# loop-Z/omniisaacgymenvs_loop

Measured on NVIDIA B200. Metric: ASV env-steps/sec, higher is better.
Workload: dtype f32

## Files before the change

omniisaacgymenvs_loop_b200/csrc/usv_step.cu:

```cuda
#include "usv_step_core.cuh"

namespace usv {

constexpr int kBlock = 128, kMinB = 7;
constexpr double kResidentL2Share = 0.75;

__device__ __forceinline__ void post_classic(EnvState& e, const EnvConst& k, const UsvStepParams& p, bool do_reset,
                                             bool first_call, const DynOut& s, StepOut& o, const int what = USV_CXY_ALL) {
  const float pxn = s.pxn, pyn = s.pyn, vxn = s.vxn, vyn = s.vyn, wn = s.wn, yawn = s.yawn, hs = s.hs, hc = s.hc;
  const float pa0 = s.pa0, pa1 = s.pa1;
  const float ex = k.tx - pxn, ey = k.ty - pyn;
  const float theta = wrap_pi(yawn);
  const float beta = fast_atan2(ey, ex);
  const float xa = beta - theta + USV_PI_F;
  const float alpha = ((xa >= USV_2PI_F) ? xa - USV_2PI_F : xa) - USV_PI_F;
  const float herr = fabsf(alpha);
  const float d = sqrtf(ex * ex + ey * ey);
  const float inv_d = (d > 0.0f) ? __fdividef(1.0f, d) : 0.0f;
  const float cb = (d > 0.0f) ? ex * inv_d : 1.0f, sb = ey * inv_d;
  const float ca = cb * hc + sb * hs, sa = sb * hc - cb * hs;
  o.obs[0] = hc * vxn + hs * vyn;
  o.obs[1] = -hs * vxn + hc * vyn;
  o.obs[2] = wn;
  o.obs[3] = ca;
  o.obs[4] = sa;
  o.obs[5] = d;
  o.obs[6] = vxn;
  o.obs[7] = vyn;
  o.obs[8] = 0.0f;
  o.obs[9] = vxn;
  o.obs[10] = vyn;
  o.obs[11] = 0.0f;
  o.obs[12] = 0.0f;
  const float speed = sqrtf(vxn * vxn + vyn * vyn);
  const int goal = (d < p.position_tolerance) && (speed < p.goal_speed_gate);
  if (what & USV_CXY_REWARD) e.goal_cnt = e.goal_cnt * goal + goal;
  float dist_rew;
  if (p.reward_mode == USV_REWARD_LINEAR) {
    dist_rew = p.position_scale * (e.prev_d - d);
  } else if (p.reward_mode == USV_REWARD_SQUARE) {
    dist_rew = p.position_scale * (e.prev_d * e.prev_d - d * d);
  } else {
    dist_rew = p.position_scale * (expf(-d / p.exponential_reward_coeff) - expf(-e.prev_d / p.exponential_reward_coeff));
  }
  const float h2 = herr * herr;
  const float align = p.align_la1 * (__expf(p.align_la2 * (h2 * h2)) + __expf(p.align_la3 * h2));
  if (do_reset) dist_rew = 0.0f;
  float speed_rew;
  const float sclamp = 1.0f - fminf(fmaxf(speed / 1.0f, 0.0f), 1.0f);
  if (d > 3.5f) {
    const bool in_range = (speed >= 0.8f) && (speed <= 1.5f);
    const float ds = speed - 1.15f;
    speed_rew = in_range ? 0.1f : __expf(-(ds * ds) * 5.0f) * 0.1f;
  } else if (d > 2.5f) {
    speed_rew = sclamp * 0.15f;
  } else if (d > 1.5f) {
    speed_rew = sclamp * 0.25f;
  } else {
    speed_rew = sclamp * 0.35f;
  }
  if (!(d == d)) speed_rew = 0.0f;
  const float goal_rew = (float)e.goal_cnt * p.goal_reward;
  const float task_rew = dist_rew + align + speed_rew + goal_rew + p.time_reward;
  if (what & USV_CXY_REWARD) e.prev_d = d;
  const float asum = pa0 + pa1;
  const float dw = first_call ? 0.0f : (wn - e.prev_w);
  const float dasum = first_call ? 0.0f : (asum - e.prev_asum);
  float pen_lin = 0.0f, pen_ang = 0.0f, pen_angvar = 0.0f, pen_energy = 0.0f, pen_actvar = 0.0f;
  if (p.pen_linear_vel.form != USV_PEN_OFF) pen_lin = penalty_scalar(p.pen_linear_vel, speed);
  if (p.pen_angular_vel.form != USV_PEN_OFF) pen_ang = penalty_scalar(p.pen_angular_vel, wn);
  if (p.pen_angular_vel_variation.form != USV_PEN_OFF) pen_angvar = penalty_scalar(p.pen_angular_vel_variation, dw);
  if (p.pen_energy.form == USV_PEN_NEG_SUM) pen_energy = -(pa0 + pa1) * p.pen_energy.c1 + p.pen_energy.c2;
  else if (p.pen_energy.form == USV_PEN_EXP_NEG_SUMSQ) pen_energy = (__expf(-(pa0 * pa0 + pa1 * pa1)) - 1.0f) * p.pen_energy.c1;
  if (p.pen_action_variation.form != USV_PEN_OFF) pen_actvar = penalty_scalar(p.pen_action_variation, dasum);
  const float penalties = pen_lin + pen_ang + pen_angvar + pen_energy + pen_actvar;
  if (what & USV_CXY_PENALTY) {
    e.prev_w = wn;
    e.prev_asum = asum;
  }
  o.task_rew = task_rew;
  o.penalty = penalties;
  o.rew = task_rew + penalties;
  int die = (d > p.kill_dist) ? 1 : 0;
  if ((e.goal_cnt >= p.kill_after_n_steps_in_tolerance) && (speed < p.goal_speed_gate)) die = 1;
  o.die = die;
  o.done = (e.progress >= p.max_episode_length - 1) ? 1 : die;
  o.dist_rew = dist_rew; o.align_rew = align; o.speed_rew = speed_rew; o.d = d; o.speed = speed;
  o.bdist = d - p.kill_dist;
  o.bpen = -expf(-o.bdist / 0.25f) * p.boundary_cost;
  o.pen_lin = pen_lin; o.pen_ang = pen_ang; o.pen_angvar = pen_angvar; o.pen_energy = pen_energy; o.pen_actvar = pen_actvar;
  o.absw = fabsf(wn); o.asum = asum;
  float chk = o.rew * 0.0f;
#pragma unroll
  for (int j = 0; j < kObs; ++j) chk = fmaf(o.obs[j], 0.0f, chk);
  o.finite = (chk == 0.0f);
#pragma unroll
  for (int j = 0; j < kObs; ++j)
    if (j != 8 && j != 11 && j != 12) o.obs[j] = fminf(fmaxf(o.obs[j], -p.clip_obs), p.clip_obs);
}

template <int kDisturb, bool kLutGlobal>
__device__ __forceinline__ void control_step(EnvState& e, EnvConst& k, const UsvStepParams& p, bool do_reset,
                                             float2 act, uint64_t gid, int64_t lid, uint64_t step, bool first_call,
                                             const float* __restrict__ s_lutL, const float* __restrict__ s_lutR,
                                             StepOut& o) {
  DynOut s;
  step_dynamics<kDisturb, kLutGlobal>(e, k, p, do_reset, act, gid, lid, step, s_lutL, s_lutR, s);
  post_classic(e, k, p, do_reset, first_call, s, o);
}

__device__ __forceinline__ void accumulate_stats(float* __restrict__ st0, int64_t i0, bool was_reset,
                                                 const StepOut& o, const UsvStepParams& p) {
  float* __restrict__ st = st0 + tile_base(i0, USV_ST_COUNT);
  const float v[USV_ST_COUNT] = {o.dist_rew, o.align_rew, o.speed_rew, o.d, o.speed, o.bpen, o.bdist,
                                 o.pen_lin, o.pen_ang, o.pen_angvar, o.pen_energy, o.pen_actvar,
                                 o.speed, o.absw, o.asum};
#pragma unroll
  for (int f = 0; f < USV_ST_COUNT; ++f) {
    const float prev = was_reset ? 0.0f : st[f * kTile];
    st[f * kTile] = prev + v[f];
  }
}


template <Cache C = Cache::kNormal>
__device__ __forceinline__ void write_obs_tile(float* s_obs, const StepOut& o, bool active, float* __restrict__ obs,
                                               int64_t block_start, int64_t n) {
  const int lane = threadIdx.x & 31, warp = threadIdx.x >> 5;
  float* sw = s_obs + warp * (32 * kObs);
  if (active) {
#pragma unroll
    for (int j = 0; j < kObs; ++j) sw[lane * kObs + j] = o.obs[j];
  }
  __syncwarp();
  const int64_t warp_start = block_start + (int64_t)warp * 32;
  if (warp_start >= n) return;
  const int rows = (int)min((int64_t)32, n - warp_start);
  const int total = rows * kObs;
  float* g = obs + warp_start * kObs;
  if (rows == 32 && (((uintptr_t)g & 15) == 0)) {
    const float4* s4 = reinterpret_cast<const float4*>(sw);
    float4* g4 = reinterpret_cast<float4*>(g);
#pragma unroll
    for (int q = lane; q < (32 * kObs) / 4; q += 32) st<C>(g4 + q, s4[q]);
  } else {
    for (int q = lane; q < total; q += 32) st<C>(g + q, sw[q]);
  }
  __syncwarp();
}

template <int kDisturb, bool kStats, Cache kOnePass>
__global__ void __launch_bounds__(kBlock, kMinB) step_fused_kernel(UsvEnvBuffers b, const float2* __restrict__ actions,
                                                            float* __restrict__ obs, float* __restrict__ rew,
                                                            int64_t n, const __grid_constant__ UsvStepParams p) {
  extern __shared__ __align__(16) float smem[];
  float* s_obs = smem;
  const float* __restrict__ s_lutL = b.lut_left;
  const float* __restrict__ s_lutR = b.lut_right;
  const int64_t block_start = (int64_t)blockIdx.x * kBlock;
  const int64_t i = block_start + threadIdx.x;
  const bool active = i < n;
  EnvState e;
  EnvConst k;
  bool do_reset = false;
  float2 act = make_float2(0.f, 0.f);
  if (active) {
    load_state(b.state, i, e);
    load_consts<kDisturb, kOnePass>(b.consts, i, k);
    do_reset = b.reset_buf[i] != 0;
    act = ld<kOnePass>(actions + i);
  }
  StepOut o;
  if (active) {
    control_step<kDisturb, true>(e, k, p, do_reset, act, (uint64_t)(p.env_id_offset + i), i, p.step_counter + (b.step_offset ? *b.step_offset : 0ull),
                                 p.first_call != 0, s_lutL, s_lutR, o);
    store_state(b.state, i, e);
    if (do_reset) store_consts<kDisturb, kOnePass>(b.consts, i, k);
    if (kStats) accumulate_stats(b.stats, i, do_reset, o, p);
    st<kOnePass>(rew + i, o.rew);
    b.reset_buf[i] = (int64_t)o.done;
    if (b.nonfinite_flag) {
      if (!o.finite) atomicOr(b.nonfinite_flag, 1u);
      if (!isfinite(act.x) || !isfinite(act.y)) atomicOr(b.nonfinite_flag, 2u);
    }
  }
  write_obs_tile<kOnePass>(s_obs, o, active, obs, block_start, n);
}

template <int kDisturb, bool kStats>
__global__ void __launch_bounds__(kBlock) rollout_fused_kernel(UsvEnvBuffers b, const float2* __restrict__ actions,
                                                               float* __restrict__ obs, float* __restrict__ rew,
                                                               int64_t* __restrict__ done, int T, int64_t n,
                                                               const __grid_constant__ UsvStepParams p) {
  extern __shared__ __align__(16) float smem[];
  float* s_obs = smem;
  float* s_lutL = smem + kBlock * kObs;
  float* s_lutR = s_lutL + p.n_lut;
  for (int t = threadIdx.x; t < p.n_lut; t += kBlock) {
    s_lutL[t] = b.lut_left[t];
    s_lutR[t] = b.lut_right[t];
  }
  const int64_t block_start = (int64_t)blockIdx.x * kBlock;
  const int64_t i = block_start + threadIdx.x;
  const bool active = i < n;
  EnvState e;
  EnvConst k;
  bool do_reset = false;
  bool consts_dirty = false;
  if (active) {
    load_state(b.state, i, e);
    load_consts<kDisturb>(b.consts, i, k);
    do_reset = b.reset_buf[i] != 0;
  }
  __syncthreads();
  bool first_call = p.first_call != 0;
  bool bad = false;
  const uint64_t step0 = p.step_counter + (b.step_offset ? *b.step_offset : 0ull);
  for (int t = 0; t < T; ++t) {
    StepOut o;
    if (active) {
      const float2 act = actions[(int64_t)t * n + i];
      control_step<kDisturb, false>(e, k, p, do_reset, act, (uint64_t)(p.env_id_offset + i), i, step0 + (uint64_t)t,
                             first_call, s_lutL, s_lutR, o);
      consts_dirty |= do_reset;
      if (kStats) accumulate_stats(b.stats, i, do_reset, o, p);
      if (rew) rew[(int64_t)t * n + i] = o.rew;
      if (done) done[(int64_t)t * n + i] = (int64_t)o.done;
      bad |= !o.finite || !isfinite(act.x) || !isfinite(act.y);
      do_reset = o.done != 0;
    }
    first_call = false;
    if (obs) {
      write_obs_tile(s_obs, o, active, obs + (int64_t)t * n * kObs, block_start, n);
    }
  }
  if (active) {
    store_state(b.state, i, e);
    if (consts_dirty) store_consts<kDisturb>(b.consts, i, k);
    b.reset_buf[i] = do_reset ? 1 : 0;
    if (b.nonfinite_flag && bad) atomicOr(b.nonfinite_flag, 1u);
  }
}

template <int kDisturb>
__global__ void __launch_bounds__(kBlock) planar_forces_kernel(UsvEnvBuffers b, float* __restrict__ out, int64_t n,
                                                               const __grid_constant__ UsvStepParams p) {
  const int64_t i = (int64_t)blockIdx.x * kBlock + threadIdx.x;
  if (i >= n) return;
  EnvState e;
  EnvConst k;
  load_state(b.state, i, e);
  load_consts<kDisturb>(b.consts, i, k);
  float ox = 0.0f, oy = 0.0f;
  if (kDisturb && p.envs_per_row > 0) {
    ox = p.grid_row_offset - (float)(int)(i / p.envs_per_row) * p.env_spacing;
    oy = (float)(int)(i % p.envs_per_row) * p.env_spacing - p.grid_col_offset;
  }
  float du, dv, dr, Fx, Fy, Tz, ax, ay, rdot, hsn, hcs;
  fsincos(e.psi, &hsn, &hcs);
  planar_wrench<kDisturb>(e, k, p, make_damp(k, p), ox, oy, 1.0f / k.mass, 1.0f / (p.izz * k.kiz), hsn, hcs, du, dv, dr, Fx, Fy, Tz, ax, ay, rdot);
  float* o = out + i * 8;
  o[0] = du; o[1] = dv; o[2] = dr; o[3] = Fx; o[4] = Fy; o[5] = Tz; o[6] = ax; o[7] = ay;
}

static size_t step_smem(const UsvStepParams* p) { return (size_t)(kBlock * kObs + 2 * p->n_lut) * sizeof(float); }
static size_t step_smem_nolut() { return (size_t)(kBlock * kObs) * sizeof(float); }

__global__ void __launch_bounds__(256) capturexy_task_kernel(UsvCaptureXYIO io, int64_t n, UsvStepParams p) {
  const int64_t i = (int64_t)blockIdx.x * blockDim.x + threadIdx.x;
  if (i >= n) return;
  const float2 z2 = make_float2(0.f, 0.f);
  const float2 pos = io.position ? reinterpret_cast<const float2*>(io.position)[i] : z2;
  const float2 hd = io.heading ? reinterpret_cast<const float2*>(io.heading)[i] : make_float2(1.f, 0.f);
  const float2 vel = io.linear_velocity ? reinterpret_cast<const float2*>(io.linear_velocity)[i] : z2;
  const float2 act = io.actions ? reinterpret_cast<const float2*>(io.actions)[i] : z2;
  const float2 tgt = io.target ? reinterpret_cast<const float2*>(io.target)[i] : z2;
  DynOut s;
  s.pxn = pos.x; s.pyn = pos.y; s.vxn = vel.x; s.vyn = vel.y;
  s.wn = io.angular_velocity ? io.angular_velocity[i] : 0.f;
  s.hc = hd.x; s.hs = hd.y;
  s.yawn = fast_atan2(hd.y, hd.x);
  s.pa0 = act.x; s.pa1 = act.y;
  s.raw0 = s.raw1 = s.t0 = s.t1 = s.c0 = s.c1 = 0.f;
  EnvState e;
  e.x = pos.x; e.y = pos.y; e.psi = s.yawn; e.vx = vel.x; e.vy = vel.y; e.r = s.wn; e.thrL = e.thrR = 0.f;
  e.progress = 0;
  e.goal_cnt = io.goal_reached ? io.goal_reached[i] : 0;
  const bool jr = io.just_reset ? io.just_reset[i] != 0 : false;
  EnvConst k;
  k.tx = tgt.x; k.ty = tgt.y;
  if (io.first_reward || !io.prev_position_dist) {
    const float ex = tgt.x - pos.x, ey = tgt.y - pos.y;
    e.prev_d = sqrtf(ex * ex + ey * ey);
  } else {
    e.prev_d = io.prev_position_dist[i];
  }
  e.prev_w = io.prev_angular_velocity ? io.prev_angular_velocity[i] : 0.f;
  e.prev_asum = io.prev_action_sum ? io.prev_action_sum[i] : 0.f;
  p.kill_dist = io.kill_dist;
  p.max_episode_length = 0x7fffffff;
  StepOut o;
  post_classic(e, k, p, jr, io.first_penalty != 0, s, o, io.what);
  if ((io.what & USV_CXY_OBS) && io.obs) {
#pragma unroll
    for (int j = 0; j < kObs; ++j) io.obs[i * kObs + j] = o.obs[j];
  }
  if (io.what & USV_CXY_REWARD) {
    if (io.reward) io.reward[i] = o.task_rew;
    if (io.reward_terms) { io.reward_terms[i * 3] = o.dist_rew; io.reward_terms[i * 3 + 1] = o.align_rew; io.reward_terms[i * 3 + 2] = o.speed_rew; }
    if (io.goal_reached) io.goal_reached[i] = e.goal_cnt;
    if (io.prev_position_dist) io.prev_position_dist[i] = e.prev_d;
  }
  if (io.what & USV_CXY_PENALTY) {
    if (io.penalty) io.penalty[i] = o.penalty;
    if (io.penalty_terms) {
      io.penalty_terms[i * 5] = o.pen_lin; io.penalty_terms[i * 5 + 1] = o.pen_ang; io.penalty_terms[i * 5 + 2] = o.pen_angvar;
      io.penalty_terms[i * 5 + 3] = o.pen_energy; io.penalty_terms[i * 5 + 4] = o.pen_actvar;
    }
    if (io.prev_angular_velocity) io.prev_angular_velocity[i] = e.prev_w;
    if (io.prev_action_sum) io.prev_action_sum[i] = e.prev_asum;
  }
  if ((io.what & USV_CXY_KILLS) && io.die) io.die[i] = o.die;
}

}

using namespace usv;

extern "C" {

int usv_capturexy_obs_reward_done_f32(const UsvCaptureXYIO* io, int64_t n, const UsvStepParams* p, void* stream) {
  if (!io || !p) return USV_E_NULL;
  if (n < 0) return USV_E_SIZE;
  if (n == 0) return USV_OK;
  if (!(io->what & USV_CXY_ALL) || (io->what & ~USV_CXY_ALL)) return USV_E_PARAM;
  if (!io->position || !io->target || !io->linear_velocity) return USV_E_NULL;
  if ((io->what & USV_CXY_OBS) && (!io->obs || !io->heading || !io->angular_velocity)) return USV_E_NULL;
  if ((io->what & USV_CXY_REWARD) && (!io->reward || !io->heading || !io->goal_reached)) return USV_E_NULL;
  if ((io->what & USV_CXY_PENALTY) && (!io->penalty || !io->actions || !io->angular_velocity)) return USV_E_NULL;
  if ((io->what & USV_CXY_KILLS) && (!io->die || !io->goal_reached)) return USV_E_NULL;
  const uintptr_t al = (uintptr_t)io->position | (uintptr_t)io->target | (uintptr_t)io->linear_velocity | (uintptr_t)io->heading |
                       (uintptr_t)io->actions;
  if (al & 7) return USV_E_ALIGN;
  capturexy_task_kernel<<<grid_for(n, 256), 256, 0, (cudaStream_t)stream>>>(*io, n, *p);
  return finish_launch();
}

int usv_step_fused_f32(const UsvEnvBuffers* b, const float* actions, float* obs, float* rew, int64_t n,
                       const UsvStepParams* p, void* stream) {
  int rc = check_common(b, n, p);
  if (rc) return rc;
  if (n == 0) return USV_OK;
  if (!actions || !obs || !rew) return USV_E_NULL;
  if ((uintptr_t)actions & 7) return USV_E_ALIGN;
  const size_t smem = step_smem_nolut();
  const int grid = grid_for(n, kBlock);
  const bool dis = wants_disturb(p), st = b->stats != nullptr;
  cudaStream_t s = (cudaStream_t)stream;
  const double reread = (double)n * (USV_S_COUNT * 4 + 8 + (st ? USV_ST_COUNT * 4 : 0));
  const bool one_pass_cs = reread <= kResidentL2Share * l2_bytes();
#define USV_LAUNCH_STEP(D, S)                                                                                                       \
  do {                                                                                                                              \
    auto* kern = one_pass_cs ? step_fused_kernel<D, S, Cache::kStream> : step_fused_kernel<D, S, Cache::kNormal>;                       \
    ensure_dynamic_smem(kern, smem);                                                                                                \
    kern<<<grid, kBlock, smem, s>>>(*b, (const float2*)actions, obs, rew, n, *p);                                                   \
  } while (0)
  const bool all4 = p->use_const_force && p->use_sin_force && p->use_const_torque && p->use_sin_torque && !p->use_water_current;
  if (dis && all4 && !st) USV_LAUNCH_STEP(2, false);
  else if (dis && st) USV_LAUNCH_STEP(1, true);
  else if (dis) USV_LAUNCH_STEP(1, false);
  else if (st) USV_LAUNCH_STEP(0, true);
  else USV_LAUNCH_STEP(0, false);
#undef USV_LAUNCH_STEP
  return finish_launch();
}

int usv_rollout_fused_f32(const UsvEnvBuffers* b, const float* actions, float* obs, float* rew, int64_t* done,
                          int32_t T, int64_t n, const UsvStepParams* p, void* stream) {
  int rc = check_common(b, n, p);
  if (rc) return rc;
  if (T < 0) return USV_E_SIZE;
  if (n == 0 || T == 0) return USV_OK;
  if (!actions) return USV_E_NULL;
  if ((uintptr_t)actions & 7) return USV_E_ALIGN;
  const size_t smem = step_smem(p);
  const int grid = grid_for(n, kBlock);
  const bool dis = wants_disturb(p), st = b->stats != nullptr;
  cudaStream_t s = (cudaStream_t)stream;
#define USV_LAUNCH_ROLL(D, S)                                                                              \
  do {                                                                                                     \
    ensure_dynamic_smem(rollout_fused_kernel<D, S>, smem);                                                 \
    rollout_fused_kernel<D, S><<<grid, kBlock, smem, s>>>(*b, (const float2*)actions, obs, rew, done, T, n, *p); \
  } while (0)
  if (dis && st) USV_LAUNCH_ROLL(true, true);
  else if (dis) USV_LAUNCH_ROLL(true, false);
  else if (st) USV_LAUNCH_ROLL(false, true);
  else USV_LAUNCH_ROLL(false, false);
#undef USV_LAUNCH_ROLL
  return finish_launch();
}

int usv_planar_forces_f32(const UsvEnvBuffers* b, float* out, int64_t n, const UsvStepParams* p, void* stream) {
  int rc = check_common(b, n, p);
  if (rc) return rc;
  if (n == 0) return USV_OK;
  if (!out) return USV_E_NULL;
  const int grid = grid_for(n, kBlock);
  if (wants_disturb(p))
    planar_forces_kernel<true><<<grid, kBlock, 0, (cudaStream_t)stream>>>(*b, out, n, *p);
  else
    planar_forces_kernel<false><<<grid, kBlock, 0, (cudaStream_t)stream>>>(*b, out, n, *p);
  return finish_launch();
}

}
```

omniisaacgymenvs_loop_b200/csrc/usv_step_core.cuh:

```cuda
#pragma once
#include <math_constants.h>
#include "philox.cuh"
#include "usv_common.cuh"

namespace usv {

constexpr int kObs = 13;
#define USV_PI_F 3.14159274101257324f
#define USV_2PI_F 6.28318548202514648f

struct EnvState {
  float x, y, psi, vx, vy, r, thrL, thrR, prev_d, prev_w, prev_asum;
  int goal_cnt, progress;
};
struct EnvConst {
  float tx, ty, mass, linu, linv, linr, quadu, quadv, quadr, kdrag, mL, mR, kiz;
  float fcx, fcy, fxf, fyf, fxs, fys, famp, tc, tf, ts, tamp;
};
struct StepOut {
  float obs[kObs];
  float rew, task_rew, penalty;
  int done, die;
  bool finite;
  float dist_rew, align_rew, speed_rew, d, speed, bpen, bdist;
  float pen_lin, pen_ang, pen_angvar, pen_energy, pen_actvar, absw, asum;
};

constexpr int kTile = 32;
__device__ __forceinline__ int64_t tile_base(int64_t i, int count) { return (i >> 5) * (int64_t)(count * kTile) + (i & 31); }

enum class Cache { kNormal, kStream };
template <Cache C, class T>
__device__ __forceinline__ T ld(const T* p) {
  if constexpr (C == Cache::kStream) return __ldcs(p);
  else return *p;
}
template <Cache C, class T>
__device__ __forceinline__ void st(T* p, T v) {
  if constexpr (C == Cache::kStream) __stcs(p, v);
  else *p = v;
}

__device__ __forceinline__ void load_state(const float* __restrict__ s0, int64_t i0, EnvState& e) {
  const float* __restrict__ s = s0 + tile_base(i0, USV_S_COUNT);
  e.x = s[USV_S_X * kTile];
  e.y = s[USV_S_Y * kTile];
  e.psi = s[USV_S_PSI * kTile];
  e.vx = s[USV_S_VX * kTile];
  e.vy = s[USV_S_VY * kTile];
  e.r = s[USV_S_R * kTile];
  e.thrL = s[USV_S_THR_L * kTile];
  e.thrR = s[USV_S_THR_R * kTile];
  e.prev_d = s[USV_S_PREV_D * kTile];
  e.prev_w = s[USV_S_PREV_W * kTile];
  e.prev_asum = s[USV_S_PREV_ASUM * kTile];
  e.goal_cnt = __float_as_int(s[USV_S_GOAL_CNT * kTile]);
  e.progress = __float_as_int(s[USV_S_PROGRESS * kTile]);
}

__device__ __forceinline__ void store_state(float* __restrict__ s0, int64_t i0, const EnvState& e) {
  float* __restrict__ s = s0 + tile_base(i0, USV_S_COUNT);
  s[USV_S_X * kTile] = e.x;
  s[USV_S_Y * kTile] = e.y;
  s[USV_S_PSI * kTile] = e.psi;
  s[USV_S_VX * kTile] = e.vx;
  s[USV_S_VY * kTile] = e.vy;
  s[USV_S_R * kTile] = e.r;
  s[USV_S_THR_L * kTile] = e.thrL;
  s[USV_S_THR_R * kTile] = e.thrR;
  s[USV_S_PREV_D * kTile] = e.prev_d;
  s[USV_S_PREV_W * kTile] = e.prev_w;
  s[USV_S_PREV_ASUM * kTile] = e.prev_asum;
  s[USV_S_GOAL_CNT * kTile] = __int_as_float(e.goal_cnt);
  s[USV_S_PROGRESS * kTile] = __int_as_float(e.progress);
}

template <int kDisturb, Cache C = Cache::kNormal>
__device__ __forceinline__ void load_consts(const float* __restrict__ c0, int64_t i0, EnvConst& k) {
  const float* __restrict__ c = c0 + tile_base(i0, USV_C_COUNT);
  k.tx = ld<C>(c + USV_C_TX * kTile);
  k.ty = ld<C>(c + USV_C_TY * kTile);
  k.mass = ld<C>(c + USV_C_MASS * kTile);
  k.linu = ld<C>(c + USV_C_LIN_U * kTile);
  k.linv = ld<C>(c + USV_C_LIN_V * kTile);
  k.linr = ld<C>(c + USV_C_LIN_R * kTile);
  k.quadu = ld<C>(c + USV_C_QUAD_U * kTile);
  k.quadv = ld<C>(c + USV_C_QUAD_V * kTile);
  k.quadr = ld<C>(c + USV_C_QUAD_R * kTile);
  k.kdrag = ld<C>(c + USV_C_KDRAG * kTile);
  k.mL = ld<C>(c + USV_C_THR_ML * kTile);
  k.mR = ld<C>(c + USV_C_THR_MR * kTile);
  k.kiz = ld<C>(c + USV_C_KIZ * kTile);
  if (kDisturb) {
    k.fcx = ld<C>(c + USV_C_FCX * kTile);
    k.fcy = ld<C>(c + USV_C_FCY * kTile);
    k.fxf = ld<C>(c + USV_C_FXF * kTile);
    k.fyf = ld<C>(c + USV_C_FYF * kTile);
    k.fxs = ld<C>(c + USV_C_FXS * kTile);
    k.fys = ld<C>(c + USV_C_FYS * kTile);
    k.famp = ld<C>(c + USV_C_FAMP * kTile);
    k.tc = ld<C>(c + USV_C_TC * kTile);
    k.tf = ld<C>(c + USV_C_TF * kTile);
    k.ts = ld<C>(c + USV_C_TS * kTile);
    k.tamp = ld<C>(c + USV_C_TAMP * kTile);
  } else {
    k.fcx = k.fcy = k.fxf = k.fyf = k.fxs = k.fys = k.famp = k.tc = k.tf = k.ts = k.tamp = 0.0f;
  }
}

template <int kDisturb, Cache C = Cache::kNormal>
__device__ __forceinline__ void store_consts(float* __restrict__ c0, int64_t i0, const EnvConst& k) {
  float* __restrict__ c = c0 + tile_base(i0, USV_C_COUNT);
  st<C>(c + USV_C_TX * kTile, k.tx);
  st<C>(c + USV_C_TY * kTile, k.ty);
  st<C>(c + USV_C_MASS * kTile, k.mass);
  st<C>(c + USV_C_LIN_U * kTile, k.linu);
  st<C>(c + USV_C_LIN_V * kTile, k.linv);
  st<C>(c + USV_C_LIN_R * kTile, k.linr);
  st<C>(c + USV_C_QUAD_U * kTile, k.quadu);
  st<C>(c + USV_C_QUAD_V * kTile, k.quadv);
  st<C>(c + USV_C_QUAD_R * kTile, k.quadr);
  st<C>(c + USV_C_KDRAG * kTile, k.kdrag);
  st<C>(c + USV_C_THR_ML * kTile, k.mL);
  st<C>(c + USV_C_THR_MR * kTile, k.mR);
  st<C>(c + USV_C_KIZ * kTile, k.kiz);
  if (kDisturb) {
    st<C>(c + USV_C_FCX * kTile, k.fcx);
    st<C>(c + USV_C_FCY * kTile, k.fcy);
    st<C>(c + USV_C_FXF * kTile, k.fxf);
    st<C>(c + USV_C_FYF * kTile, k.fyf);
    st<C>(c + USV_C_FXS * kTile, k.fxs);
    st<C>(c + USV_C_FYS * kTile, k.fys);
    st<C>(c + USV_C_FAMP * kTile, k.famp);
    st<C>(c + USV_C_TC * kTile, k.tc);
    st<C>(c + USV_C_TF * kTile, k.tf);
    st<C>(c + USV_C_TS * kTile, k.ts);
    st<C>(c + USV_C_TAMP * kTile, k.tamp);
  }
}

__device__ __forceinline__ float urange(float u, float lo, float hi) { return u * (hi - lo) + lo; }

__device__ __forceinline__ void trig_reduce(float x, float& r, int& q) {
  const float j = rintf(x * 0.636619772f);
  q = (int)j;
  r = fmaf(j, -1.57079601e+00f, x);
  r = fmaf(j, -3.13916473e-07f, r);
  r = fmaf(j, -5.39030253e-15f, r);
}
__device__ __forceinline__ float poly_sin(float r, float r2) {
  float p = fmaf(r2, -1.9515295891e-4f, 8.3321608736e-3f);
  p = fmaf(p, r2, -1.6666654611e-1f);
  return fmaf(p * r2, r, r);
}
__device__ __forceinline__ float poly_cos(float r2) {
  float p = fmaf(r2, 2.443315711809948e-5f, -1.388731625493765e-3f);
  p = fmaf(p, r2, 4.166664568298827e-2f);
  p = fmaf(p, r2, -0.5f);
  return fmaf(p, r2, 1.0f);
}
__device__ __forceinline__ void fsincos(float x, float* sp, float* cp) {
  float r; int q;
  trig_reduce(x, r, q);
  const float r2 = r * r;
  const float s = poly_sin(r, r2), c = poly_cos(r2);
  const float ss = (q & 1) ? c : s;
  const float cc = (q & 1) ? s : c;
  *sp = __int_as_float(__float_as_int(ss) ^ ((q & 2) << 30));
  *cp = __int_as_float(__float_as_int(cc) ^ (((q + 1) & 2) << 30));
}
__device__ __forceinline__ float fsin_sfu(float x) {
  const float k = rintf(x * 0.159154943f);
  float r = fmaf(k, -6.28318548e+00f, x);
  r = fmaf(k, 1.74845553e-07f, r);
  return __sinf(r);
}
__device__ __forceinline__ float fsin(float x) {
  float r; int q;
  trig_reduce(x, r, q);
  const float r2 = r * r;
  const float v = (q & 1) ? poly_cos(r2) : poly_sin(r, r2);
  return __int_as_float(__float_as_int(v) ^ ((q & 2) << 30));
}

__device__ __forceinline__ float fast_atan2(float y, float x) {
  const float ax = fabsf(x), ay = fabsf(y);
  const float mx = fmaxf(ax, ay), mn = fminf(ax, ay);
  const float t = (mx > 0.0f) ? __fdividef(mn, mx) : 0.0f;
  const float t2 = t * t;
  float p = fmaf(t2, -0.00455979211255908f, 0.023780519142746925f);
  p = fmaf(p, t2, -0.05882975459098816f);
  p = fmaf(p, t2, 0.09868865460157394f);
  p = fmaf(p, t2, -0.14003290235996246f);
  p = fmaf(p, t2, 0.19966961443424225f);
  p = fmaf(p, t2, -0.3333181142807007f);
  p = fmaf(p, t2, 0.9999998807907104f);
  float a = p * t;
  a = (ay > ax) ? 1.57079637f - a : a;
  a = (x < 0.0f) ? 3.14159274f - a : a;
  return (y < 0.0f) ? -a : a;
}

__device__ __forceinline__ float wrap_pi(float a) {
  a = a - USV_2PI_F * rintf(a * (1.0f / USV_2PI_F));
  a = (a > USV_PI_F) ? a - USV_2PI_F : a;
  a = (a <= -USV_PI_F) ? a + USV_2PI_F : a;
  return a;
}

__device__ __forceinline__ float penalty_scalar(const UsvPenaltyTerm& t, float x) {
  switch (t.form) {
    case USV_PEN_NEG_ABS: return -fabsf(x) * t.c1 + t.c2;
    case USV_PEN_NEG_DEADZONE: return -fmaxf(fabsf(x) - t.k, 0.0f) * t.c1;
    case USV_PEN_EXP_NEG_ABS: return (__expf(-t.k * fabsf(x)) - 1.0f) * t.c1;
    default: return 0.0f;
  }
}

__device__ __forceinline__ void spawn_xy(const UsvStepParams& p, const Uniform4& r0, float tx, float ty, float& x, float& y) {
  const float sr = r0.c * (p.spawn_max_dist - p.spawn_min_dist) + p.spawn_min_dist;
  const float sth = r0.d * 2.0f * USV_PI_F;
  float ssp, csp;
  fsincos(sth, &ssp, &csp);
  x = p.spawn_about_origin ? sr * csp : sr * csp + tx;
  y = p.spawn_about_origin ? sr * ssp : sr * ssp + ty;
}

template <int kDisturb>
__device__ __forceinline__ void reset_env(EnvState& e, EnvConst& k, const UsvStepParams& p, uint64_t gid, uint64_t step) {
  const Uniform4 r0 = philox_uniform4(p.seed, gid, step, RS_RESET_0);
  const Uniform4 r1 = philox_uniform4(p.seed, gid, step, RS_RESET_1);
  e.goal_cnt = 0;
  if (kDisturb) {
    if (p.use_force_disturbance) {
      const Uniform4 r5 = philox_uniform4(p.seed, gid, step, RS_RESET_5);
      const Uniform4 r6 = philox_uniform4(p.seed, gid, step, RS_RESET_6);
      const Uniform4 r7 = philox_uniform4(p.seed, gid, step, RS_RESET_7);
      if (p.use_sin_force) {
        k.fxf = urange(r5.c, p.force_min_freq, p.force_max_freq);
        k.fyf = urange(r5.d, p.force_min_freq, p.force_max_freq);
        k.fxs = urange(r6.a, p.force_min_shift, p.force_max_shift);
        k.fys = urange(r6.b, p.force_min_shift, p.force_max_shift);
        k.famp = urange(r6.c, p.force_sin_min, p.force_sin_max);
      }
      if (p.use_const_force) {
        const float rr = urange(r6.d, p.force_const_min, p.force_const_max);
        const float th = r7.a * USV_PI_F * 2.0f;
        float sth_, cth_;
        fsincos(th, &sth_, &cth_);
        k.fcx = cth_ * rr;
        k.fcy = sth_ * rr;
      }
    }
    if (p.use_torque_disturbance) {
      const Uniform4 r7 = philox_uniform4(p.seed, gid, step, RS_RESET_7);
      const Uniform4 r8 = philox_uniform4(p.seed, gid, step, RS_RESET_8);
      if (p.use_sin_torque) {
        k.tf = urange(r7.b, p.torque_min_freq, p.torque_max_freq);
        k.ts = urange(r7.c, p.torque_min_shift, p.torque_max_shift);
        k.tamp = urange(r7.d, p.torque_sin_min, p.torque_sin_max);
      }
      if (p.use_const_torque) {
        float rr = urange(r8.a, p.torque_const_min, p.torque_const_max);
        if (r8.b > 0.5f) rr *= -1.0f;
        k.tc = rr;
      }
    }
  }
  k.mass = p.mass_rand ? urange(r1.d, p.mass_min, p.mass_max) : p.mass_base;
  if (p.kiz_rand && !(p.mass_coupling && (p.couple_targets & 4))) {
    const Uniform4 r5 = philox_uniform4(p.seed, gid, step, RS_RESET_5);
    if (p.kiz_log) {
      const float l0 = logf(p.couple_kiz_min), l1 = logf(p.couple_kiz_max);
      k.kiz = expf(l0 + r5.b * (l1 - l0));
    } else {
      k.kiz = p.couple_kiz_min + r5.b * (p.couple_kiz_max - p.couple_kiz_min);
    }
  }
  if (p.drag_rand) {
    const Uniform4 r3 = philox_uniform4(p.seed, gid, step, RS_RESET_3);
    const Uniform4 r4 = philox_uniform4(p.seed, gid, step, RS_RESET_4);
    k.linu = p.lin_base[0] + (r3.a * 2.0f - 1.0f) * p.lin_rand[0];
    k.linv = p.lin_base[1] + (r3.b * 2.0f - 1.0f) * p.lin_rand[1];
    k.linr = p.lin_base[2] + (r3.c * 2.0f - 1.0f) * p.lin_rand[2];
    k.quadu = p.quad_base[0] + (r4.a * 2.0f - 1.0f) * p.quad_rand[0];
    k.quadv = p.quad_base[1] + (r4.b * 2.0f - 1.0f) * p.quad_rand[1];
    k.quadr = p.quad_base[2] + (r4.c * 2.0f - 1.0f) * p.quad_rand[2];
  }
  if (p.kdrag_rand) {
    const Uniform4 r2 = philox_uniform4(p.seed, gid, step, RS_RESET_2);
    if (p.kdrag_log) {
      const float l0 = logf(p.kdrag_min), l1 = logf(p.kdrag_max);
      k.kdrag = expf(l0 + r2.d * (l1 - l0));
    } else {
      k.kdrag = p.kdrag_min + r2.d * (p.kdrag_max - p.kdrag_min);
    }
  }
  if (p.thr_rand) {
    if (p.thr_separate) {
      const Uniform4 r4 = philox_uniform4(p.seed, gid, step, RS_RESET_4);
      const Uniform4 r5 = philox_uniform4(p.seed, gid, step, RS_RESET_5);
      k.mL = r4.d * 2.0f * p.thr_left_frac + (1.0f - p.thr_left_frac);
      k.mR = r5.a * 2.0f * p.thr_right_frac + (1.0f - p.thr_right_frac);
    } else {
      const Uniform4 r3 = philox_uniform4(p.seed, gid, step, RS_RESET_3);
      k.mL = k.mR = r3.d * 2.0f * p.thr_rand_frac + (1.0f - p.thr_rand_frac);
    }
  }
  if (p.mass_coupling) {
    const float denom = fmaxf(p.couple_mass_max - p.mass_base, 1e-6f);
    const float rr = fminf(fmaxf((k.mass - p.mass_base) / denom, 0.0f), 1.0f);
    if (p.couple_targets & 1) k.kdrag = p.kdrag_min + rr * (p.kdrag_max - p.kdrag_min);
    if (p.couple_targets & 2) {
      const float s = fminf(fmaxf(1.0f - rr * p.couple_thr_a, 1.0f - p.couple_thr_a), 1.0f);
      k.mL = k.mR = s;
    }
    if (p.couple_targets & 4) k.kiz = p.couple_kiz_min + rr * (p.couple_kiz_max - p.couple_kiz_min);
  }
  if (!p.reset_pose_external) {
    if (p.retarget_after_spawn) spawn_xy(p, r0, k.tx, k.ty, e.x, e.y);
    if (p.retarget_on_reset) {
      k.tx = r0.a * p.goal_random_position * 2.0f - p.goal_random_position;
      k.ty = r0.b * p.goal_random_position * 2.0f - p.goal_random_position;
    }
    if (!p.retarget_after_spawn) spawn_xy(p, r0, k.tx, k.ty, e.x, e.y);
    e.psi = r1.a * USV_PI_F;
    e.vx = r1.b * (2.0f * p.spawn_vel_range) - p.spawn_vel_range;
    e.vy = r1.c * (2.0f * p.spawn_vel_range) - p.spawn_vel_range;
    e.r = 0.0f;
  }
  e.progress = 0;
}

struct Damp { float au, bu, av, bv, ar, br; };
__device__ __forceinline__ Damp make_damp(const EnvConst& k, const UsvStepParams& p) {
  const float sc = p.use_drag_scale ? p.scaling_damping * k.kdrag : p.scaling_damping;
  const float off_fwd = p.offset_lin_forward_damping_speed;
  Damp d;
  d.au = ((k.linu + p.offset_linear_damping) - (p.lin_fwd[0] + off_fwd)) * sc;
  d.av = ((k.linv + p.offset_linear_damping) - (p.lin_fwd[1] + off_fwd)) * sc;
  d.ar = ((k.linr + p.offset_linear_damping) - (p.lin_fwd[2] + off_fwd)) * sc;
  d.bu = (k.quadu + p.offset_nonlin_damping) * sc;
  d.bv = (k.quadv + p.offset_nonlin_damping) * sc;
  d.br = (k.quadr + p.offset_nonlin_damping) * sc;
  return d;
}

template <int kDisturb>
__device__ __forceinline__ void planar_wrench(const EnvState& e, const EnvConst& k, const UsvStepParams& p, const Damp& dm, float ox,
                                              float oy, float inv_m, float inv_iz, float s, float c, float& du, float& dv,
                                              float& dr, float& Fx, float& Fy, float& Tz, float& ax, float& ay,
                                              float& rdot) {
  float u = c * e.vx + s * e.vy;
  float v = -s * e.vx + c * e.vy;
  const float w = e.r;
  if (kDisturb == 1 && p.use_water_current) {
    u -= c * p.flow_vel_xy[0] + s * p.flow_vel_xy[1];
    v -= -s * p.flow_vel_xy[0] + c * p.flow_vel_xy[1];
  }
  du = -fmaf(dm.bu, fabsf(u), dm.au) * u;
  dv = -fmaf(dm.bv, fabsf(v), dm.av) * v;
  dr = -fmaf(dm.br, fabsf(w), dm.ar) * w;
  float fdx = 0.0f, fdy = 0.0f, td = 0.0f;
  if (kDisturb) {
    const bool cf = kDisturb == 2 || p.use_const_force, sf = kDisturb == 2 || p.use_sin_force;
    const bool ct = kDisturb == 2 || p.use_const_torque, stq = kDisturb == 2 || p.use_sin_torque;
    if (cf) { fdx = k.fcx; fdy = k.fcy; }
    if (sf) {
      fdx = k.fcx + fsin_sfu((e.x + ox) * k.fxf + k.fxs) * k.famp;
      fdy = k.fcy + fsin_sfu((e.y + oy) * k.fyf + k.fys) * k.famp;
    }
    if (ct) td = k.tc;
    if (stq) td = k.tc + fsin_sfu(((e.x + ox) + (e.y + oy)) * k.tf + k.ts) * k.tamp;
  }
  Fx = fdx + du + e.thrL + e.thrR;
  Fy = fdy + dv;
  Tz = td + dr - p.thr_y_left * e.thrL - p.thr_y_right * e.thrR;
  ax = (c * Fx - s * Fy) * inv_m;
  ay = (s * Fx + c * Fy) * inv_m;
  rdot = Tz * inv_iz;
}

struct DynOut {
  float raw0, raw1;
  float pa0, pa1;
  float t0, t1;
  float c0, c1;
  float pxn, pyn, vxn, vyn, wn, yawn, hs, hc;
};

template <int kDisturb, bool kLutGlobal>
__device__ __forceinline__ void step_dynamics(EnvState& e, EnvConst& k, const UsvStepParams& p, bool do_reset,
                                             float2 act, uint64_t gid, int64_t lid, uint64_t step,
                                             const float* __restrict__ s_lutL, const float* __restrict__ s_lutR,
                                             DynOut& s) {
  if (do_reset) reset_env<kDisturb>(e, k, p, gid, step);
  const Uniform8 nz = philox_uniform8x16(p.seed, gid, step, RS_STEP_A);
  const float u_a0 = nz.v[0], u_a1 = nz.v[1], u_vx = nz.v[2], u_vy = nz.v[3], u_w = nz.v[4], u_h = nz.v[5],
              u_px = nz.v[6], u_py = nz.v[7];
  float a0 = fminf(fmaxf(act.x, -p.clip_actions), p.clip_actions);
  float a1 = fminf(fmaxf(act.y, -p.clip_actions), p.clip_actions);
  float pa0, pa1;
  float c0, c1;
  s.raw0 = a0; s.raw1 = a1;
  if (!p.action_affine) {
    if (p.action_noise) {
      a0 += urange(u_a0, p.action_noise_min, p.action_noise_max);
      a1 += urange(u_a1, p.action_noise_min, p.action_noise_max);
    }
    pa0 = a0; pa1 = a1;
    c0 = fminf(fmaxf(a0, -1.0f), 1.0f);
    c1 = fminf(fmaxf(a1, -1.0f), 1.0f);
    s.t0 = c0; s.t1 = c1;
  } else {
    float t0 = a0 + p.action_bias, t1 = a1 + p.action_bias;
    if (p.action_noise) {
      t0 += urange(u_a0, p.action_noise_min, p.action_noise_max);
      t1 += urange(u_a1, p.action_noise_min, p.action_noise_max);
    }
    t0 = fminf(fmaxf(t0, -1.0f), 1.0f);
    t1 = fminf(fmaxf(t1, -1.0f), 1.0f);
    s.t0 = t0; s.t1 = t1;
    c0 = fminf(fmaxf(0.5f * (t0 + 1.0f), 0.0f), 1.0f);
    c1 = fminf(fmaxf(0.5f * (t1 + 1.0f), 0.0f), 1.0f);
    pa0 = p.penalties_use_u ? c0 : a0;
    pa1 = p.penalties_use_u ? c1 : a1;
  }
  s.pa0 = pa0; s.pa1 = pa1; s.c0 = c0; s.c1 = c1;
  if (do_reset) { c0 = 0.0f; c1 = 0.0f; }
  const int iL = lut_index(c0, p.n_lut), iR = lut_index(c1, p.n_lut);
  const float tgtL = (kLutGlobal ? __ldg(s_lutL + iL) : s_lutL[iL]) * k.mL;
  const float tgtR = (kLutGlobal ? __ldg(s_lutR + iR) : s_lutR[iR]) * k.mR;

  float ox = 0.0f, oy = 0.0f;
  if (kDisturb && p.envs_per_row > 0) {
    const int row = (int)(lid / p.envs_per_row), col = (int)(lid % p.envs_per_row);
    ox = p.grid_row_offset - (float)row * p.env_spacing;
    oy = (float)col * p.env_spacing - p.grid_col_offset;
  }
  const float oma = 1.0f - p.lag_alpha;
  const float inv_m = __fdividef(1.0f, k.mass), inv_iz = __fdividef(1.0f, p.izz * k.kiz);
  float hsn, hcs;
  fsincos(e.psi, &hsn, &hcs);
  const Damp dm = make_damp(k, p);
  for (int ss = 0; ss < p.n_substeps; ++ss) {
    e.thrL = __fadd_rn(__fmul_rn(e.thrL, p.lag_alpha), __fmul_rn(oma, tgtL));
    e.thrR = __fadd_rn(__fmul_rn(e.thrR, p.lag_alpha), __fmul_rn(oma, tgtR));
    float du, dv, dr, Fx, Fy, Tz, ax, ay, rdot;
    planar_wrench<kDisturb>(e, k, p, dm, ox, oy, inv_m, inv_iz, hsn, hcs, du, dv, dr, Fx, Fy, Tz, ax, ay, rdot);
    e.vx += p.dt * ax;
    e.vy += p.dt * ay;
    e.r += p.dt * rdot;
    e.x += p.dt * e.vx;
    e.y += p.dt * e.vy;
    const float dpsi = p.dt * e.r;
    e.psi += dpsi;
    if (fabsf(dpsi) <= 0.0625f) {
      const float d2 = dpsi * dpsi;
      const float sd = dpsi * fmaf(d2, fmaf(d2, 1.0f / 120.0f, -1.0f / 6.0f), 1.0f);
      const float cd = fmaf(d2, fmaf(d2, 1.0f / 24.0f, -0.5f), 1.0f);
      const float nc = hcs * cd - hsn * sd;
      hsn = hsn * cd + hcs * sd;
      hcs = nc;
    } else {
      fsincos(e.psi, &hsn, &hcs);
    }
  }
  e.psi = wrap_pi(e.psi);

  e.progress += 1;
  float pxn = e.x, pyn = e.y, vxn = e.vx, vyn = e.vy, wn = e.r, yawn = e.psi;
  if (p.noise_pos) { pxn += urange(u_px, p.pos_noise_min, p.pos_noise_max); pyn += urange(u_py, p.pos_noise_min, p.pos_noise_max); }
  if (p.noise_vel) {
    vxn += urange(u_vx, p.vel_noise_min, p.vel_noise_max);
    vyn += urange(u_vy, p.vel_noise_min, p.vel_noise_max);
    wn += urange(u_w, p.vel_noise_min, p.vel_noise_max);
  }
  float hs = hsn, hc = hcs;
  if (p.noise_heading) {
    const float dh = urange(u_h, p.heading_noise_min, p.heading_noise_max);
    yawn += dh;
    if (fabsf(dh) <= 0.5f) {
      const float d2 = dh * dh;
      const float sd = dh * fmaf(d2, fmaf(d2, fmaf(d2, -1.0f / 5040.0f, 1.0f / 120.0f), -1.0f / 6.0f), 1.0f);
      const float cd = fmaf(d2, fmaf(d2, fmaf(d2, fmaf(d2, 1.0f / 40320.0f, -1.0f / 720.0f), 1.0f / 24.0f), -0.5f), 1.0f);
      hc = hcs * cd - hsn * sd;
      hs = hsn * cd + hcs * sd;
    } else {
      fsincos(yawn, &hs, &hc);
    }
  }
  s.pxn = pxn; s.pyn = pyn; s.vxn = vxn; s.vyn = vyn; s.wn = wn; s.yawn = yawn; s.hs = hs; s.hc = hc;
}

inline int check_common(const UsvEnvBuffers* b, int64_t n, const UsvStepParams* p) {
  if (!b || !p) return USV_E_NULL;
  if (n < 0) return USV_E_SIZE;
  if (!b->state || !b->consts || !b->reset_buf || !b->lut_left || !b->lut_right) return USV_E_NULL;
  if (b->state_stride < n || b->consts_stride < n || (b->state_stride & 31) || (b->consts_stride & 31)) return USV_E_SIZE;
  if (b->stats && (b->stats_stride < n || (b->stats_stride & 31))) return USV_E_SIZE;
  if (p->n_lut < 2 || p->n_lut > 8192) return USV_E_PARAM;
  if (p->n_substeps < 0 || p->n_substeps > 1024) return USV_E_PARAM;
  if (!(p->izz > 0.0f)) return USV_E_PARAM;
  if (p->reward_mode < USV_REWARD_LINEAR || p->reward_mode > USV_REWARD_EXPONENTIAL) return USV_E_PARAM;
  return USV_OK;
}

inline bool wants_disturb(const UsvStepParams* p) {
  return p->use_force_disturbance || p->use_torque_disturbance || p->use_const_force || p->use_sin_force ||
         p->use_const_torque || p->use_sin_torque || p->use_water_current;
}

}
```

Before: 22.11 billion.

## Use packed float2 math in planar dynamics and unroll fixed five-substep loop

Rewrites the planar wrench and substep integration to use packed f32x2 intrinsics (__ffma2_rn, __fmul2_rn, __fadd2_rn), pairing the x/y computations. Adds a compile-time substep count template so the common five-substep disturbed path runs a fully unrolled loop. Together these aim to cut instruction count in the inner integration loop. The cost is more register pressure from unrolling and possible small rounding differences from reordered fused operations.

```diff
diff --git a/omniisaacgymenvs_loop_b200/csrc/usv_step.cu b/omniisaacgymenvs_loop_b200/csrc/usv_step.cu
--- a/omniisaacgymenvs_loop_b200/csrc/usv_step.cu
+++ b/omniisaacgymenvs_loop_b200/csrc/usv_step.cu
@@ -99,13 +99,13 @@
     if (j != 8 && j != 11 && j != 12) o.obs[j] = fminf(fmaxf(o.obs[j], -p.clip_obs), p.clip_obs);
 }
 
-template <int kDisturb, bool kLutGlobal>
+template <int kDisturb, bool kLutGlobal, int kSubsteps = 0>
 __device__ __forceinline__ void control_step(EnvState& e, EnvConst& k, const UsvStepParams& p, bool do_reset,
                                              float2 act, uint64_t gid, int64_t lid, uint64_t step, bool first_call,
                                              const float* __restrict__ s_lutL, const float* __restrict__ s_lutR,
                                              StepOut& o) {
   DynOut s;
-  step_dynamics<kDisturb, kLutGlobal>(e, k, p, do_reset, act, gid, lid, step, s_lutL, s_lutR, s);
+  step_dynamics<kDisturb, kLutGlobal, kSubsteps>(e, k, p, do_reset, act, gid, lid, step, s_lutL, s_lutR, s);
   post_classic(e, k, p, do_reset, first_call, s, o);
 }
 
@@ -149,7 +149,7 @@
   __syncwarp();
 }
 
-template <int kDisturb, bool kStats, Cache kOnePass>
+template <int kDisturb, bool kStats, Cache kOnePass, int kSubsteps = 0>
 __global__ void __launch_bounds__(kBlock, kMinB) step_fused_kernel(UsvEnvBuffers b, const float2* __restrict__ actions,
                                                             float* __restrict__ obs, float* __restrict__ rew,
                                                             int64_t n, const __grid_constant__ UsvStepParams p) {
@@ -172,7 +172,7 @@
   }
   StepOut o;
   if (active) {
-    control_step<kDisturb, true>(e, k, p, do_reset, act, (uint64_t)(p.env_id_offset + i), i, p.step_counter + (b.step_offset ? *b.step_offset : 0ull),
+    control_step<kDisturb, true, kSubsteps>(e, k, p, do_reset, act, (uint64_t)(p.env_id_offset + i), i, p.step_counter + (b.step_offset ? *b.step_offset : 0ull),
                                  p.first_call != 0, s_lutL, s_lutR, o);
     store_state(b.state, i, e);
     if (do_reset) store_consts<kDisturb, kOnePass>(b.consts, i, k);
@@ -251,16 +251,18 @@
   EnvConst k;
   load_state(b.state, i, e);
   load_consts<kDisturb>(b.consts, i, k);
-  float ox = 0.0f, oy = 0.0f;
+  float2 off = make_float2(0.0f, 0.0f);
   if (kDisturb && p.envs_per_row > 0) {
-    ox = p.grid_row_offset - (float)(int)(i / p.envs_per_row) * p.env_spacing;
-    oy = (float)(int)(i % p.envs_per_row) * p.env_spacing - p.grid_col_offset;
-  }
-  float du, dv, dr, Fx, Fy, Tz, ax, ay, rdot, hsn, hcs;
-  fsincos(e.psi, &hsn, &hcs);
-  planar_wrench<kDisturb>(e, k, p, make_damp(k, p), ox, oy, 1.0f / k.mass, 1.0f / (p.izz * k.kiz), hsn, hcs, du, dv, dr, Fx, Fy, Tz, ax, ay, rdot);
+    off.x = p.grid_row_offset - (float)(int)(i / p.envs_per_row) * p.env_spacing;
+    off.y = (float)(int)(i % p.envs_per_row) * p.env_spacing - p.grid_col_offset;
+  }
+  float2 h, uv, dcoef, F, acc;
+  float dr, Tz, rdot;
+  fsincos(e.psi, &h.y, &h.x);
+  planar_wrench<kDisturb>(e, make_float2(e.x, e.y), make_float2(e.vx, e.vy), k, p, make_damp(k, p), off, 1.0f / k.mass,
+                          1.0f / (p.izz * k.kiz), h, uv, dcoef, dr, F, Tz, acc, rdot);
   float* o = out + i * 8;
-  o[0] = du; o[1] = dv; o[2] = dr; o[3] = Fx; o[4] = Fy; o[5] = Tz; o[6] = ax; o[7] = ay;
+  o[0] = -dcoef.x * uv.x; o[1] = -dcoef.y * uv.y; o[2] = dr; o[3] = F.x; o[4] = F.y; o[5] = Tz; o[6] = acc.x; o[7] = acc.y;
 }
 
 static size_t step_smem(const UsvStepParams* p) { return (size_t)(kBlock * kObs + 2 * p->n_lut) * sizeof(float); }
@@ -359,18 +361,19 @@
   cudaStream_t s = (cudaStream_t)stream;
   const double reread = (double)n * (USV_S_COUNT * 4 + 8 + (st ? USV_ST_COUNT * 4 : 0));
   const bool one_pass_cs = reread <= kResidentL2Share * l2_bytes();
-#define USV_LAUNCH_STEP(D, S)                                                                                                       \
+#define USV_LAUNCH_STEP(D, S, N)                                                                                                    \
   do {                                                                                                                              \
-    auto* kern = one_pass_cs ? step_fused_kernel<D, S, Cache::kStream> : step_fused_kernel<D, S, Cache::kNormal>;                       \
+    auto* kern = one_pass_cs ? step_fused_kernel<D, S, Cache::kStream, N> : step_fused_kernel<D, S, Cache::kNormal, N>;             \
     ensure_dynamic_smem(kern, smem);                                                                                                \
     kern<<<grid, kBlock, smem, s>>>(*b, (const float2*)actions, obs, rew, n, *p);                                                   \
   } while (0)
   const bool all4 = p->use_const_force && p->use_sin_force && p->use_const_torque && p->use_sin_torque && !p->use_water_current;
-  if (dis && all4 && !st) USV_LAUNCH_STEP(2, false);
-  else if (dis && st) USV_LAUNCH_STEP(1, true);
-  else if (dis) USV_LAUNCH_STEP(1, false);
-  else if (st) USV_LAUNCH_STEP(0, true);
-  else USV_LAUNCH_STEP(0, false);
+  if (dis && all4 && !st && p->n_substeps == 5) USV_LAUNCH_STEP(2, false, 5);
+  else if (dis && all4 && !st) USV_LAUNCH_STEP(2, false, 0);
+  else if (dis && st) USV_LAUNCH_STEP(1, true, 0);
+  else if (dis) USV_LAUNCH_STEP(1, false, 0);
+  else if (st) USV_LAUNCH_STEP(0, true, 0);
+  else USV_LAUNCH_STEP(0, false, 0);
 #undef USV_LAUNCH_STEP
   return finish_launch();
 }
diff --git a/omniisaacgymenvs_loop_b200/csrc/usv_step_core.cuh b/omniisaacgymenvs_loop_b200/csrc/usv_step_core.cuh
--- a/omniisaacgymenvs_loop_b200/csrc/usv_step_core.cuh
+++ b/omniisaacgymenvs_loop_b200/csrc/usv_step_core.cuh
@@ -6,6 +6,8 @@
 namespace usv {
 
 constexpr int kObs = 13;
+
+__device__ __forceinline__ float2 bcast2(float v) { return make_float2(v, v); }
 #define USV_PI_F 3.14159274101257324f
 #define USV_2PI_F 6.28318548202514648f
 
@@ -175,6 +177,13 @@
   r = fmaf(k, 1.74845553e-07f, r);
   return __sinf(r);
 }
+__device__ __forceinline__ float2 fsin_sfu2(float2 x) {
+  const float2 j = __fmul2_rn(x, bcast2(0.159154943f));
+  const float2 k = make_float2(rintf(j.x), rintf(j.y));
+  float2 r = __ffma2_rn(k, bcast2(-6.28318548e+00f), x);
+  r = __ffma2_rn(k, bcast2(1.74845553e-07f), r);
+  return make_float2(__sinf(r.x), __sinf(r.y));
+}
 __device__ __forceinline__ float fsin(float x) {
   float r; int q;
   trig_reduce(x, r, q);
@@ -332,52 +341,51 @@
   e.progress = 0;
 }
 
-struct Damp { float au, bu, av, bv, ar, br; };
+struct Damp { float2 a, b; float ar, br; };
 __device__ __forceinline__ Damp make_damp(const EnvConst& k, const UsvStepParams& p) {
   const float sc = p.use_drag_scale ? p.scaling_damping * k.kdrag : p.scaling_damping;
   const float off_fwd = p.offset_lin_forward_damping_speed;
   Damp d;
-  d.au = ((k.linu + p.offset_linear_damping) - (p.lin_fwd[0] + off_fwd)) * sc;
-  d.av = ((k.linv + p.offset_linear_damping) - (p.lin_fwd[1] + off_fwd)) * sc;
+  d.a.x = ((k.linu + p.offset_linear_damping) - (p.lin_fwd[0] + off_fwd)) * sc;
+  d.a.y = ((k.linv + p.offset_linear_damping) - (p.lin_fwd[1] + off_fwd)) * sc;
   d.ar = ((k.linr + p.offset_linear_damping) - (p.lin_fwd[2] + off_fwd)) * sc;
-  d.bu = (k.quadu + p.offset_nonlin_damping) * sc;
-  d.bv = (k.quadv + p.offset_nonlin_damping) * sc;
+  d.b.x = (k.quadu + p.offset_nonlin_damping) * sc;
+  d.b.y = (k.quadv + p.offset_nonlin_damping) * sc;
   d.br = (k.quadr + p.offset_nonlin_damping) * sc;
   return d;
 }
 
 template <int kDisturb>
-__device__ __forceinline__ void planar_wrench(const EnvState& e, const EnvConst& k, const UsvStepParams& p, const Damp& dm, float ox,
-                                              float oy, float inv_m, float inv_iz, float s, float c, float& du, float& dv,
-                                              float& dr, float& Fx, float& Fy, float& Tz, float& ax, float& ay,
-                                              float& rdot) {
-  float u = c * e.vx + s * e.vy;
-  float v = -s * e.vx + c * e.vy;
+__device__ __forceinline__ void planar_wrench(const EnvState& e, float2 pos, float2 vel, const EnvConst& k, const UsvStepParams& p,
+                                              const Damp& dm, float2 off, float inv_m, float inv_iz, float2 h, float2& uv,
+                                              float2& dcoef, float& dr, float2& F, float& Tz, float2& acc, float& rdot) {
+  const float c = h.x, s = h.y;
+  uv = __ffma2_rn(make_float2(s, c), bcast2(vel.y), __fmul2_rn(make_float2(c, -s), bcast2(vel.x)));
   const float w = e.r;
   if (kDisturb == 1 && p.use_water_current) {
-    u -= c * p.flow_vel_xy[0] + s * p.flow_vel_xy[1];
-    v -= -s * p.flow_vel_xy[0] + c * p.flow_vel_xy[1];
-  }
-  du = -fmaf(dm.bu, fabsf(u), dm.au) * u;
-  dv = -fmaf(dm.bv, fabsf(v), dm.av) * v;
+    uv.x -= c * p.flow_vel_xy[0] + s * p.flow_vel_xy[1];
+    uv.y -= -s * p.flow_vel_xy[0] + c * p.flow_vel_xy[1];
+  }
+  dcoef = __ffma2_rn(make_float2(fabsf(uv.x), fabsf(uv.y)), dm.b, dm.a);
   dr = -fmaf(dm.br, fabsf(w), dm.ar) * w;
-  float fdx = 0.0f, fdy = 0.0f, td = 0.0f;
+  float2 fd = make_float2(0.0f, 0.0f);
+  float td = 0.0f;
   if (kDisturb) {
     const bool cf = kDisturb == 2 || p.use_const_force, sf = kDisturb == 2 || p.use_sin_force;
     const bool ct = kDisturb == 2 || p.use_const_torque, stq = kDisturb == 2 || p.use_sin_torque;
-    if (cf) { fdx = k.fcx; fdy = k.fcy; }
+    const float2 wp = __fadd2_rn(pos, off);
+    if (cf) fd = make_float2(k.fcx, k.fcy);
     if (sf) {
-      fdx = k.fcx + fsin_sfu((e.x + ox) * k.fxf + k.fxs) * k.famp;
-      fdy = k.fcy + fsin_sfu((e.y + oy) * k.fyf + k.fys) * k.famp;
+      const float2 ph = __ffma2_rn(wp, make_float2(k.fxf, k.fyf), make_float2(k.fxs, k.fys));
+      fd = __ffma2_rn(fsin_sfu2(ph), bcast2(k.famp), make_float2(k.fcx, k.fcy));
     }
     if (ct) td = k.tc;
-    if (stq) td = k.tc + fsin_sfu(((e.x + ox) + (e.y + oy)) * k.tf + k.ts) * k.tamp;
-  }
-  Fx = fdx + du + e.thrL + e.thrR;
-  Fy = fdy + dv;
+    if (stq) td = k.tc + fsin_sfu((wp.x + wp.y) * k.tf + k.ts) * k.tamp;
+  }
+  F = __ffma2_rn(make_float2(-uv.x, -uv.y), dcoef, fd);
+  F.x = F.x + e.thrL + e.thrR;
   Tz = td + dr - p.thr_y_left * e.thrL - p.thr_y_right * e.thrR;
-  ax = (c * Fx - s * Fy) * inv_m;
-  ay = (s * Fx + c * Fy) * inv_m;
+  acc = __fmul2_rn(__ffma2_rn(F, bcast2(c), __fmul2_rn(make_float2(-F.y, F.x), bcast2(s))), bcast2(inv_m));
   rdot = Tz * inv_iz;
 }
 
@@ -389,7 +397,7 @@
   float pxn, pyn, vxn, vyn, wn, yawn, hs, hc;
 };
 
-template <int kDisturb, bool kLutGlobal>
+template <int kDisturb, bool kLutGlobal, int kSubsteps = 0>
 __device__ __forceinline__ void step_dynamics(EnvState& e, EnvConst& k, const UsvStepParams& p, bool do_reset,
                                              float2 act, uint64_t gid, int64_t lid, uint64_t step,
                                              const float* __restrict__ s_lutL, const float* __restrict__ s_lutR,
@@ -432,41 +440,49 @@
   const float tgtL = (kLutGlobal ? __ldg(s_lutL + iL) : s_lutL[iL]) * k.mL;
   const float tgtR = (kLutGlobal ? __ldg(s_lutR + iR) : s_lutR[iR]) * k.mR;
 
-  float ox = 0.0f, oy = 0.0f;
+  float2 off = make_float2(0.0f, 0.0f);
   if (kDisturb && p.envs_per_row > 0) {
     const int row = (int)(lid / p.envs_per_row), col = (int)(lid % p.envs_per_row);
-    ox = p.grid_row_offset - (float)row * p.env_spacing;
-    oy = (float)col * p.env_spacing - p.grid_col_offset;
+    off.x = p.grid_row_offset - (float)row * p.env_spacing;
+    off.y = (float)col * p.env_spacing - p.grid_col_offset;
   }
   const float oma = 1.0f - p.lag_alpha;
   const float inv_m = __fdividef(1.0f, k.mass), inv_iz = __fdividef(1.0f, p.izz * k.kiz);
-  float hsn, hcs;
-  fsincos(e.psi, &hsn, &hcs);
+  float2 h;
+  fsincos(e.psi, &h.y, &h.x);
   const Damp dm = make_damp(k, p);
-  for (int ss = 0; ss < p.n_substeps; ++ss) {
+  float2 pos = make_float2(e.x, e.y), vel = make_float2(e.vx, e.vy);
+  auto substep = [&]() {
     e.thrL = __fadd_rn(__fmul_rn(e.thrL, p.lag_alpha), __fmul_rn(oma, tgtL));
     e.thrR = __fadd_rn(__fmul_rn(e.thrR, p.lag_alpha), __fmul_rn(oma, tgtR));
-    float du, dv, dr, Fx, Fy, Tz, ax, ay, rdot;
-    planar_wrench<kDisturb>(e, k, p, dm, ox, oy, inv_m, inv_iz, hsn, hcs, du, dv, dr, Fx, Fy, Tz, ax, ay, rdot);
-    e.vx += p.dt * ax;
-    e.vy += p.dt * ay;
+    float2 uv, dcoef, F, acc;
+    float dr, Tz, rdot;
+    planar_wrench<kDisturb>(e, pos, vel, k, p, dm, off, inv_m, inv_iz, h, uv, dcoef, dr, F, Tz, acc, rdot);
+    vel = __ffma2_rn(acc, bcast2(p.dt), vel);
     e.r += p.dt * rdot;
-    e.x += p.dt * e.vx;
-    e.y += p.dt * e.vy;
+    pos = __ffma2_rn(vel, bcast2(p.dt), pos);
     const float dpsi = p.dt * e.r;
     e.psi += dpsi;
     if (fabsf(dpsi) <= 0.0625f) {
       const float d2 = dpsi * dpsi;
       const float sd = dpsi * fmaf(d2, fmaf(d2, 1.0f / 120.0f, -1.0f / 6.0f), 1.0f);
       const float cd = fmaf(d2, fmaf(d2, 1.0f / 24.0f, -0.5f), 1.0f);
-      const float nc = hcs * cd - hsn * sd;
-      hsn = hsn * cd + hcs * sd;
-      hcs = nc;
+      const float nc = h.x * cd - h.y * sd;
+      h.y = h.y * cd + h.x * sd;
+      h.x = nc;
     } else {
-      fsincos(e.psi, &hsn, &hcs);
-    }
-  }
+      fsincos(e.psi, &h.y, &h.x);
+    }
+  };
+  if constexpr (kSubsteps > 0) {
+#pragma unroll
+    for (int ss = 0; ss < kSubsteps; ++ss) substep();
+  } else {
+    for (int ss = 0; ss < p.n_substeps; ++ss) substep();
+  }
+  e.x = pos.x; e.y = pos.y; e.vx = vel.x; e.vy = vel.y;
   e.psi = wrap_pi(e.psi);
+  const float hsn = h.y, hcs = h.x;
 
   e.progress += 1;
   float pxn = e.x, pyn = e.y, vxn = e.vx, vyn = e.vy, wn = e.r, yawn = e.psi;
```

Result: faster. 22.38 billion, median of 6 (+1.2%).
